# hherlyng/knp-emi-cgx

Measured on AMD Instinct MI355X. Metric: MDoF/s per implicit timestep (assembly+GMRES), higher is better.
Workload: dtype f64

## Files before the change

include/knpemi_hip.h:

```cpp
#ifndef KNPEMI_HIP_H
#define KNPEMI_HIP_H

#include <stdint.h>

#ifdef __cplusplus
extern "C" {
#endif

#define KNP_MAX_IONS 3
#define KNP_MAX_AUX 8
#define KNP_DIAG_MAX_CONSTS 64
#define KNP_MAX_PROG_REGS 48
#define KNP_STATE_MAX_INSTR 768
#define KNP_STATE_MAX_CONSTS 128
#define KNP_MAX_AMG_LEVELS 16
#define KNP_FUNCTIONAL_MAX_Q 125

#define KNP_OK 0
#define KNP_E_ARG (-1)
#define KNP_E_HIP (-2)
#define KNP_E_STATE (-3)
#define KNP_E_ALLOC (-4)
#define KNP_E_MESH (-5)

// ... 241 lines not shown
int knp_timer_read(knp_ctx* ctx, int32_t capacity, double* seconds , int32_t* n_intervals);
int knp_timer_pending(const knp_ctx* ctx);
int knp_profile_enable(knp_ctx* ctx, int32_t class_mask);
int knp_profile_get(knp_ctx* ctx, int32_t cls, double* ms, int64_t* launches);
int knp_profile_reset(knp_ctx* ctx);
enum { KNP_ST_BNORM = 0 , KNP_ST_ALLREDUCE = 1 ,
       KNP_ST_HALO = 2 , KNP_ST_READBACK = 3 ,
       KNP_ST_FUSED = 4 ,
       KNP_ST_NORM_FALLBACK = 5 ,
       KNP_ST_BLOCKED = 6 ,
       KNP_ST_FUSED_LEVELS = 7 ,
       KNP_ST_FUSED_DOTS = 8 ,
       KNP_ST_SPMV_DOTS = 9 ,
       KNP_ST_FUSED_TAILS = 10 ,
       KNP_ST_KNOD_SKIPS = 11 ,
       KNP_ST_COUNT = 12 };
int knp_get_stats(const knp_ctx* ctx, double* out );
int knp_get_traffic_model(const knp_ctx* ctx, double* out );
enum { KNP_LI_ASM_VARIANT = 0 ,
       KNP_LI_ASM_STAGE = 1 ,
       KNP_LI_ASM_DMAX = 2 ,
       KNP_LI_ASM_GROUP = 3, KNP_LI_SPMV_GROUP = 4, KNP_LI_PC_GROUP = 5 ,
       KNP_LI_MAX_NODE_CELLS = 6 ,
       KNP_LI_MAX_NODE_PAIRS = 7 ,
       KNP_LI_SPMV_UNROLL = 8 ,
       KNP_LI_SPMV_MK = 9 ,
       KNP_LI_COUNT = 10 };
int knp_get_launch_info(const knp_ctx* ctx, int32_t* out , int n);
enum { KNP_AI_A_LANES = 0, KNP_AI_P_LANES = 1, KNP_AI_R_LANES = 2, KNP_AI_S_LANES = 3, KNP_AI_RT_LANES = 4, KNP_AI_U_LANES = 5,
       KNP_AI_BA_LANES = 6, KNP_AI_BR_LANES = 7, KNP_AI_BS_LANES = 8, KNP_AI_BRT_LANES = 9, KNP_AI_BU_LANES = 10,
       KNP_AI_P_N_ACT = 11, KNP_AI_S_N_ACT = 12 ,
// ... 13 lines not shown
```

knp-emi-cgx_amd/cgx_hip/backend.py:

```python
from __future__ import annotations

import ctypes as C
import os

import numpy as np
import torch

from . import _lib
from ._lib import Fields, FieldsOut, KnpError, MeshDesc
from .parallel import HaloPlan, all_reduce_sum_, guarded


class _CAI:

    def __init__(self, ptr, n):
        self.__cuda_array_interface__ = {"shape": (int(n),), "typestr": "<f8", "data": (int(ptr), False),
                                         "version": 2, "strides": None}


def _f64(a):
    return a.ctypes.data_as(_lib.f64p)


def _i32(a):
# ... 673 lines not shown
                k = C.c_int32()
                self.check(self.lib.knp_timer_read(self.ctx, 1, out, C.byref(k)))
            return np.zeros(0)
        out = (C.c_double * n)()
        k = C.c_int32()
        self.check(self.lib.knp_timer_read(self.ctx, n, out, C.byref(k)))
        return np.array(out[:k.value], dtype=np.float64)

    def profile_enable(self, mask=0x1f):
        self.check(self.lib.knp_profile_enable(self.ctx, int(mask)))

    def profile_reset(self):
        self.check(self.lib.knp_profile_reset(self.ctx))

    def stats(self):
        out = (C.c_double * 12)()
        self.check(self.lib.knp_get_stats(self.ctx, out))
        return {"bnorm": out[0], "allreduces": int(out[1]), "halos": int(out[2]), "readbacks": int(out[3]), "fused": int(out[4]),
                "norm_fallbacks": int(out[5]), "blocked": int(out[6]), "fused_levels": int(out[7]),
                "fused_dots": int(out[8]), "spmv_dots": int(out[9]), "fused_tails": int(out[10]), "knod_skips": int(out[11])}

    def nodal_conc(self):
        out = np.empty((self.n_nodes, 4), dtype=np.float64)
        self.check(self.lib.knp_get_nodal_conc(self.ctx, _f64(out)))
        return out

    def traffic_model(self):
        out = (C.c_double * 5)()
        self.check(self.lib.knp_get_traffic_model(self.ctx, out))
        return {"spmv": out[0], "pc": out[1], "assembly_matrix": out[2], "assembly_rhs": out[3], "vector": out[4]}

    def launch_info(self):
        names = ["asm_variant", "asm_stage", "asm_dmax", "asm_group", "spmv_group", "pc_group", "max_node_cells", "max_node_pairs",
                 "spmv_unroll", "spmv_mk"]
        out = (C.c_int32 * len(names))()
# ... 21 lines not shown
```

knp-emi-cgx_amd/csrc/knp_internal.hpp:

```cpp
#pragma once
#include <hip/hip_runtime.h>

#include <cstdint>
#include <string>
#include <vector>

#include "knpemi_hip.h"

#define KNP_NPROF 5

struct KnpHostGraph {
    int dim = 0, nv1 = 0;
    int n_v = 0, n_v_owned = 0, n_c = 0, n_c_owned = 0, n_g = 0, n_q = 0;
    int n_nodes = 0, n_nodes_owned = 0;
    std::vector<int32_t> node_i, node_e;
    std::vector<int32_t> node_vertex;
    std::vector<uint8_t> node_side;
    std::vector<int32_t> pair_ptr;
    std::vector<int32_t> pair_col;
    std::vector<int32_t> pair_row;
    std::vector<double> pair_M, pair_K;
    std::vector<int32_t> contrib_ptr;
    std::vector<int32_t> contrib_cell;
    std::vector<double> contrib_k;
// ... 363 lines not shown
    bool asm_pending = false;
    double last_bnorm = 0.0;
    int64_t n_allreduce = 0, n_halo = 0, n_readback = 0;
    int64_t n_fused_dots = 0;
    int64_t n_spmv_dots = 0;
    int fused_tail = 1;
    int update_early = 1;
    bool tail_ok = false;
    bool have_tail_target = false;
    knp_fields_out tail_target = {};
    const double* tail_x = nullptr;
    bool fields_current = false, knod_current = false, fields_promise = false;
    bool knod_skipped = false;
    int64_t n_fused_tail = 0;
    int64_t n_knod_skip = 0;
    std::vector<hipEvent_t> tm_events;
    size_t tm_used = 0;
    KnpDiagMap diag_cells, diag_facets;
    KnpDiagMap diag_flux;
    double2* d_flux_rec = nullptr;
    KnpDiagMap diag_phim;
    int32_t* diag_code = nullptr;
    int diag_n_instr = 0, diag_n_regs = 0, diag_n_consts = 0;
    double diag_consts[KNP_DIAG_MAX_CONSTS] = {};
    bool diag_prog = false;
    KnpEmi emi;
    KnpStates states;
    std::vector<KnpSamplePlan> sample_plans;
    std::vector<KnpFunctional> functionals;
    std::vector<KnpFunctional> membrane_functionals;
// ... 11 lines not shown
```

knp-emi-cgx_amd/csrc/knp_kernels.hip:

```cpp
#include <hip/hip_runtime.h>
#include <hip/hip_ext.h>

#include <algorithm>
#include <cmath>
#include <cstdio>
#include <cstdlib>
#include <cstring>
#include <new>

#include "knp_dispatch.hpp"
#include "knp_internal.hpp"

#define HIPCHK(call)                                                                       \
    do {                                                                                   \
        hipError_t e_ = (call);                                                            \
        if (e_ != hipSuccess) {                                                            \
            ctx->err = std::string(#call) + ": " + hipGetErrorString(e_);                  \
            return KNP_E_HIP;                                                              \
        }                                                                                  \
    } while (0)
#define KCHK(expr)                         \
    do {                                   \
        int rc_ = (expr);                  \
        if (rc_ != KNP_OK) return rc_;     \
// ... 14 lines not shown
    double dz2i[3], dz2e[3];
    double rFz[3], cmFz[3];
    double rF;
};
struct FieldPtrs {
    const double* ki[3];
    const double* ke[3];
    const double* phim;
    const double* aux[KNP_MAX_AUX];
};

static void side_discard(knp_ctx* ctx);
static DevParams make_params(const knp_ctx* ctx);
static int64_t phi_block_nnz(const knp_ctx* ctx);
static int join_asm(knp_ctx* ctx);
static bool fin_ok(const knp_ctx* ctx);
static hipEvent_t prof_event(knp_ctx* ctx);
static void free_hier(KnpAmgHier& H);
static inline int nblocks(int64_t n, int per = NT) { return (int)std::max<int64_t>(1, (n + per - 1) / per); }

__device__ __forceinline__ double wave_sum(double v) {
#pragma unroll
    for (int o = 32; o > 0; o >>= 1) v += __shfl_xor(v, o, 64);
    return v;
}
__device__ __forceinline__ double block_sum(double v, double* sm) {
    v = wave_sum(v);
    const int w = threadIdx.x >> 6, l = threadIdx.x & 63;
    __syncthreads();
    if (l == 0) sm[w] = v;
// ... 316 lines not shown
    for (int o = G >> 1; o > 0; o >>= 1) {
        T0 += __shfl_xor(T0, o, G);
        T1 += __shfl_xor(T1, o, G);
        T2 += __shfl_xor(T2, o, G);
    }
    if (live && selfq < 255 && (selfq & (G - 1)) == lane) emit(p0 + selfq, -T0, -T1, -T2);
}

static void launch_cell_means(knp_ctx* ctx, const FieldPtrs& f, bool matrix = false) {
    const KnpHostGraph& g = ctx->g;
    bool skip = matrix && ctx->asm_dmax > 0 && ctx->fields_promise && ctx->knod_current && ctx->have_tail_target && (ctx->prof_on & ~1) == 0;
    for (int j = 0; j < 3 && skip; ++j) skip = f.ki[j] == ctx->tail_target.k_i[j] && f.ke[j] == ctx->tail_target.k_e[j];
    ctx->fields_promise = false;
    ctx->knod_current = false;
    if (matrix) ctx->knod_skipped = skip;
    if (skip) { ++ctx->n_knod_skip; return; }
    if (ctx->asm_dmax > 0)
        hipLaunchKernelGGL(k_nodal_conc, dim3(nblocks(g.n_nodes)), dim3(NT), 0, ctx->stream, g.n_nodes, ctx->d_node_vertex, ctx->d_node_side, f, ctx->d_knod);
    else
        hipLaunchKernelGGL(k_cell_means, dim3(nblocks(g.n_c)), dim3(NT), 0, ctx->stream, g.n_c, g.nv1, ctx->d_cells, ctx->d_cell_side, f, ctx->d_cbar);
}
template <bool PRECOND, bool TD_ONLY>
static void launch_assemble_nodes(knp_ctx* ctx, const DevParams& P, double* at, double* ac) {
    const KnpHostGraph& g = ctx->g;
    const int n = g.n_nodes_owned;
    if (n <= 0) return;
    if (ctx->asm_stage > 0 && ctx->d_tc_meta) {
        const int cmax = ctx->asm_stage;
        const int dmax = ctx->asm_dmax, nv1 = g.nv1;
        with_lanes<4, 32>(ctx->asm_group, [&](auto G) { with_flag(dmax > 0, [&](auto F) {
            hipLaunchKernelGGL((k_assemble_nodes_tr<PRECOND, TD_ONLY, G(), F()>), dim3(nblocks((int64_t)n * G())), dim3(NT),
// ... 2345 lines not shown
                if (nd >= g.n_nodes || g.node_vertex[nd] != v || g.node_side[nd] != s) { ok = false; break; }
                ++hits;
            }
        ctx->tail_ok = ok && hits == g.n_nodes;
    }
    std::vector<int32_t>().swap(g.contrib_cell);
    std::vector<double>().swap(g.contrib_k);
    std::vector<int32_t>().swap(g.node_cell);
    std::vector<uint8_t>().swap(g.contrib_slot);
    return KNP_OK;
}

int knp_destroy(knp_ctx* ctx) {
    if (!ctx) return KNP_OK;
    (void)hipDeviceSynchronize();
    if (ctx->stream2) { (void)hipEventDestroy(ctx->ev_fork); (void)hipEventDestroy(ctx->ev_join); (void)hipStreamDestroy(ctx->stream2); }
    if (ctx->stream3) { (void)hipEventDestroy(ctx->ev_x); (void)hipEventDestroy(ctx->ev_halo); (void)hipStreamDestroy(ctx->stream3); }
    if (ctx->stream_asm) { (void)hipEventDestroy(ctx->ev_fork_asm); (void)hipEventDestroy(ctx->ev_asm); (void)hipStreamDestroy(ctx->stream_asm); }
    dev_free(ctx->d_t2_s); dev_free(ctx->d_w2_s); dev_free(ctx->d_wb); dev_free(ctx->d_partial_s);
    dev_free(ctx->d_nodes_int); dev_free(ctx->d_nodes_bnd);
    knp_p2p_free(ctx);
    knp_jit_release(ctx);
    for (auto& r : ctx->prof_recs) { (void)hipEventDestroy(r.a); (void)hipEventDestroy(r.b); }
    for (auto& e : ctx->prof_pool) (void)hipEventDestroy(e);
    for (auto& e : ctx->tm_events) (void)hipEventDestroy(e);
    dev_free(ctx->d_cells); dev_free(ctx->d_cell_side); dev_free(ctx->d_coords);
    dev_free(ctx->d_node_vertex); dev_free(ctx->d_node_side); dev_free(ctx->d_node_i); dev_free(ctx->d_node_e);
    dev_free(ctx->d_pair_ptr); dev_free(ctx->d_pair_col); dev_free(ctx->d_pair_row);
    dev_free(ctx->d_pair_M); dev_free(ctx->d_pair_K); dev_free(ctx->d_pair_MK);
    dev_free(ctx->d_contrib_ptr); dev_free(ctx->d_contrib_cell); dev_free(ctx->d_contrib_k);
    dev_free(ctx->d_node_cell_ptr); dev_free(ctx->d_node_cell); dev_free(ctx->d_contrib_slot); dev_free(ctx->d_ncv); dev_free(ctx->d_knod);
    dev_free(ctx->d_tc_meta); dev_free(ctx->d_tc_k); dev_free(ctx->d_tc_slot);
    dev_free(ctx->d_fv); dev_free(ctx->d_fmeas); dev_free(ctx->d_gamma_prog); dev_free(ctx->d_qp); dev_free(ctx->d_qw);
    dev_free(ctx->d_gv_vertex); dev_free(ctx->d_gv_node_i); dev_free(ctx->d_gv_node_e); dev_free(ctx->d_node_gv);
    dev_free(ctx->d_gptr); dev_free(ctx->d_gcol); dev_free(ctx->d_grow); dev_free(ctx->d_gq_i); dev_free(ctx->d_gq_e);
    dev_free(ctx->d_gdiag); dev_free(ctx->d_gcptr); dev_free(ctx->d_gc_facet); dev_free(ctx->d_gc_lab);
    dev_free(ctx->d_at); dev_free(ctx->d_ac); dev_free(ctx->d_ax); dev_free(ctx->d_gx_i); dev_free(ctx->d_gx_e);
    dev_free(ctx->d_p_vals); dev_free(ctx->d_px);
    dev_free(ctx->d_cbar); dev_free(ctx->d_fmat); dev_free(ctx->d_fvec);
    dev_free(ctx->d_partial); dev_free(ctx->d_red); dev_free(ctx->d_y); dev_free(ctx->d_vbj); dev_free(ctx->d_gm);
    if (ctx->h_red) (void)hipHostFree(ctx->h_red);
    if (ctx->h_seq) (void)hipHostFree((void*)ctx->h_seq);
    dev_free(ctx->d_V); dev_free(ctx->d_Z); dev_free(ctx->d_w); dev_free(ctx->d_t);
    for (auto& p : ctx->progs) { dev_free(p.d_code); dev_free(p.d_consts); if (p.h_consts) (void)hipHostFree(p.h_consts); }
    dev_free(ctx->d_prog_code); dev_free(ctx->d_prog_consts); dev_free(ctx->d_prog_len); dev_free(ctx->d_prog_nconsts);
    for (int h = 0; h < KNP_MAX_HIER; ++h) free_hier(ctx->hier[h]);
    dev_free(ctx->d_p_vals_f);
    dev_free(ctx->d_ML); dev_free(ctx->d_cc); dev_free(ctx->d_t2); dev_free(ctx->d_w2);
    dev_free(ctx->d_defl_mode); dev_free(ctx->d_defl_einv); dev_free(ctx->d_bc_dofs);
    knp_diag_free(ctx);
    knp_emi_free(ctx);
    knp_state_free(ctx);
// ... 114 lines not shown
    HIPCHK(hipStreamSynchronize(ctx->stream));
    HIPCHK(hipMemcpy(h.data(), ctx->d_partial, h.size() * sizeof(double), hipMemcpyDeviceToHost));
    double m = 0.0;
    for (int k = 0; k < 3; ++k)
        if (len[k] > 0)
            for (int b = 0; b < RED_BLOCKS; ++b) m = std::max(m, h[(size_t)k * RED_BLOCKS + b]);
    *out = m;
    return KNP_OK;
}

int knp_set_params(knp_ctx* ctx, double dt, double F, double C_M, double psi, int32_t n_ions, const double* z,
                   const double* Di, const double* De) {
    CHECK_CTX(ctx);
    if (n_ions != 3 || !z || !Di || !De) { ctx->err = "n_ions must be 3 (Na, K, Cl; KNPEMIx_problem.py:980-981)"; return KNP_E_ARG; }
    if (!(dt > 0) || !(psi > 0) || F == 0.0) { ctx->err = "dt, psi must be positive and F non-zero"; return KNP_E_ARG; }
    ctx->dt = dt; ctx->F = F; ctx->C_M = C_M; ctx->psi = psi; ctx->n_ions = 3;
    ctx->asm_dt = -1.0;
    for (int j = 0; j < 3; ++j) {
        if (z[j] == 0.0 || !(Di[j] > 0) || !(De[j] > 0)) { ctx->err = "valence must be non-zero and diffusivities positive"; return KNP_E_ARG; }
        ctx->z[j] = z[j]; ctx->Di[j] = Di[j]; ctx->De[j] = De[j];
    }
    return KNP_OK;
}

static int validate_program(knp_ctx* ctx, int n_instr, const int32_t* code, int n_consts, int* n_regs_out) {
    int max_reg = -1;
    for (int i = 0; i < n_instr; ++i) {
        const int op = code[4 * i], d = code[4 * i + 1], a = code[4 * i + 2], b = code[4 * i + 3];
        auto regok = [&](int r) { if (r > max_reg) max_reg = r; return r >= 0 && r < KNP_MAX_PROG_REGS; };
        bool ok = true;
// ... 77 lines not shown
int knp_set_dirichlet(knp_ctx* ctx, int32_t n, const int32_t* dofs) {
    CHECK_CTX(ctx);
    side_discard(ctx);
    if (n < 0 || (n > 0 && !dofs)) { ctx->err = "bad Dirichlet arguments"; return KNP_E_ARG; }
    for (int i = 0; i < n; ++i)
        if (dofs[i] < 0 || dofs[i] >= ctx->n_dof_owned) { ctx->err = "Dirichlet dof out of range (owned dofs only)"; return KNP_E_ARG; }
    HIPCHK(hipStreamSynchronize(ctx->stream));
    dev_free(ctx->d_bc_dofs);
    ctx->n_bc = 0;
    if (n > 0) {
        KCHK(dev_upload_raw(ctx, &ctx->d_bc_dofs, dofs, (size_t)n));
        ctx->n_bc = n;
    }
    ctx->asm_dt = -1.0;
    ctx->fields_current = ctx->knod_current = false;
    return KNP_OK;
}

int knp_set_sources(knp_ctx* ctx, const double* const* fi, const double* const* fe) {
    CHECK_CTX(ctx);
    ctx->have_sources = false;
    for (int j = 0; j < 3; ++j) {
        ctx->src_i[j] = fi ? fi[j] : nullptr;
        ctx->src_e[j] = fe ? fe[j] : nullptr;
        if (ctx->src_i[j] || ctx->src_e[j]) ctx->have_sources = true;
    }
    return KNP_OK;
}

static int check_fields(knp_ctx* ctx, const knp_fields* f, bool need_phim) {
// ... 9 lines not shown
    if (ctx->pc_kind == KNP_PC_AMG || ctx->pc_kind == KNP_PC_VBJACOBI) { ctx->have_cc = false; return; }
    const KnpHostGraph& g = ctx->g;
    hipLaunchKernelGGL(k_schur_diag, dim3(nblocks(g.n_nodes_owned)), dim3(NT), 0, ctx->stream, g.n_nodes_owned, ctx->psi, ctx->z[0], ctx->z[1],
                       ctx->z[2], ctx->d_node_vertex, ctx->d_node_side, f, ctx->d_ML, ctx->d_cc);
    ctx->have_cc = true;
}

static int join_asm(knp_ctx* ctx) {
    if (ctx->asm_pending) {
        HIPCHK(hipStreamWaitEvent(ctx->stream, ctx->ev_asm, 0));
        ctx->asm_pending = false;
    }
    return KNP_OK;
}

static int assemble_matrix_on_stream(knp_ctx* ctx, const knp_fields* fields, bool with_schur_diag) {
    const KnpHostGraph& g = ctx->g;
    const DevParams P = make_params(ctx);
    FieldPtrs f = make_fields(fields);
    ProfScope ps(ctx, 3);
    launch_cell_means(ctx, f, true);
    const bool td_only = ctx->have_A && !ctx->asm_full && ctx->asm_dt == ctx->dt;
    if (td_only) launch_assemble_nodes<false, true>(ctx, P, ctx->d_at, ctx->d_ac);
    else launch_assemble_nodes<false, false>(ctx, P, ctx->d_at, ctx->d_ac);
    ctx->asm_dt = ctx->dt;
    if (g.n_g > 0) {
        if (g.dim == 2)
            hipLaunchKernelGGL((k_gamma_facets<2, true, false, 8, 1, NT, 1>), dim3(nblocks((int64_t)g.n_g * 8)), dim3(NT), 0, ctx->stream, g.n_g, g.n_q, P,
                               ctx->d_fv, ctx->d_fmeas, ctx->d_qp, ctx->d_qw, f, 0, ctx->d_coords, ctx->d_gamma_prog,
                               (const int32_t* const*)nullptr, (const int32_t*)nullptr, (const double* const*)nullptr,
                               (const int32_t*)nullptr, 0, 0, ctx->d_fmat, ctx->d_fvec);
        else if (gamma_many(g)) {
            hipLaunchKernelGGL((k_gamma_facets<3, true, false, 4, 9, 64, 1>), dim3((unsigned)(((int64_t)g.n_g * 4 + 63) / 64)), dim3(64), 0, ctx->stream, g.n_g, g.n_q, P,
                               ctx->d_fv, ctx->d_fmeas, ctx->d_qp, ctx->d_qw, f, 0, ctx->d_coords, ctx->d_gamma_prog,
                               (const int32_t* const*)nullptr, (const int32_t*)nullptr, (const double* const*)nullptr,
                               (const int32_t*)nullptr, 0, 0, ctx->d_fmat, ctx->d_fvec);
        }
        else
            hipLaunchKernelGGL((k_gamma_facets<3, true, false, 16, 3, 64, 2>), dim3((unsigned)(((int64_t)g.n_g * 16 + 63) / 64)), dim3(64), 0, ctx->stream, g.n_g, g.n_q, P,
                               ctx->d_fv, ctx->d_fmeas, ctx->d_qp, ctx->d_qw, f, 0, ctx->d_coords, ctx->d_gamma_prog,
                               (const int32_t* const*)nullptr, (const int32_t*)nullptr, (const double* const*)nullptr,
                               (const int32_t*)nullptr, 0, 0, ctx->d_fmat, ctx->d_fvec);
        if (ctx->n_gp)
            hipLaunchKernelGGL((k_gamma_pairs<false>), dim3(nblocks(ctx->n_gp)), dim3(NT), 0, ctx->stream, ctx->n_gp, g.n_g, g.dim, P,
                               ctx->d_grow, ctx->d_gptr, ctx->d_gv_node_i, ctx->d_gv_node_e, ctx->d_gq_i, ctx->d_gq_e,
                               ctx->d_gcptr, ctx->d_gc_facet, ctx->d_gc_lab, ctx->d_fmeas, ctx->d_fmat, ctx->d_pair_ptr,
                               ctx->d_at, ctx->d_ax);
    }
    if (ctx->n_bc > 0)
        hipLaunchKernelGGL(k_dirichlet_rows_A, dim3(nblocks(ctx->n_bc)), dim3(NT), 0, ctx->stream, ctx->n_bc, ctx->d_bc_dofs, ctx->d_pair_ptr,
                           ctx->d_pair_col, ctx->d_node_gv, ctx->d_node_side, ctx->d_gptr, ctx->d_ac, ctx->d_at, ctx->d_ax);
    if (with_schur_diag && !ctx->prep.left()) launch_schur_diag(ctx, f);
    HIPCHK(hipGetLastError());
    ctx->have_A = true;
    if (ctx->pc_kind == KNP_PC_VBJACOBI) {
        hipLaunchKernelGGL(k_vbj_extract, dim3(nblocks(g.n_nodes_owned)), dim3(NT), 0, ctx->stream, g.n_nodes_owned,
                           ctx->d_pair_ptr, ctx->d_pair_col, ctx->d_ac, ctx->d_at, ctx->d_ax, ctx->d_node_gv, ctx->d_node_side,
                           ctx->d_gdiag, ctx->d_vbj);
        HIPCHK(hipGetLastError());
    }
    return KNP_OK;
}

int knp_assemble_matrix(knp_ctx* ctx, const knp_fields* fields) {
    CHECK_CTX(ctx);
    KCHK(check_fields(ctx, fields, false));
    KCHK(join_asm(ctx));
    return assemble_matrix_on_stream(ctx, fields, true);
}

int knp_assemble_matrix_async(knp_ctx* ctx, const knp_fields* fields) {
    CHECK_CTX(ctx);
    KCHK(check_fields(ctx, fields, false));
    KCHK(join_asm(ctx));
    static const bool off = getenv("KNP_ASM_ASYNC") && atoi(getenv("KNP_ASM_ASYNC")) == 0;
    if (off || ctx->pc_kind == KNP_PC_VBJACOBI || (ctx->prof_on & ~1) || !ctx->have_A || ctx->prep.left())
        return assemble_matrix_on_stream(ctx, fields, true);
    if (!ctx->stream_asm) {
        HIPCHK(hipStreamCreateWithFlags(&ctx->stream_asm, hipStreamNonBlocking));
        HIPCHK(hipEventCreateWithFlags(&ctx->ev_fork_asm, hipEventDisableTiming));
        HIPCHK(hipEventCreateWithFlags(&ctx->ev_asm, hipEventDisableTiming));
    }
    HIPCHK(hipEventRecord(ctx->ev_fork_asm, ctx->stream));
    HIPCHK(hipStreamWaitEvent(ctx->stream_asm, ctx->ev_fork_asm, 0));
    hipStream_t main_stream = ctx->stream;
    ctx->stream = ctx->stream_asm;
    const int rc = assemble_matrix_on_stream(ctx, fields, false);
    ctx->stream = main_stream;
    KCHK(rc);
    HIPCHK(hipEventRecord(ctx->ev_asm, ctx->stream_asm));
    ctx->asm_pending = true;
    return KNP_OK;
}

int knp_pc_set_coupled_potential(knp_ctx* ctx, int32_t on) {
    CHECK_CTX(ctx);
    side_discard(ctx);
    ctx->pc_coupled_phi = on ? 1 : 0;
    if (on && !ctx->d_px) {
        HIPCHK(hipMalloc((void**)&ctx->d_px, (size_t)std::max<int64_t>(ctx->n_gp, 1) * sizeof(double)));
        HIPCHK(hipMemset(ctx->d_px, 0, (size_t)std::max<int64_t>(ctx->n_gp, 1) * sizeof(double)));
    }
// ... 27 lines not shown
        rp[n] = (int32_t)k;
        for (int p = g.pair_ptr[n]; p < g.pair_ptr[n + 1]; ++p) { ci[k] = g.pair_col[p]; vals[k++] = pm[(size_t)4 * p + 3]; }
        const int A = g.node_gv[n];
        if (ctx->pc_coupled_phi && A >= 0) {
            const std::vector<int32_t>& gx = g.node_side[n] ? g.gx_e : g.gx_i;
            for (int s = g.gptr[A]; s < g.gptr[A + 1]; ++s) { ci[k] = gx[s]; vals[k++] = px[s]; }
        }
    }
    rp[g.n_nodes_owned] = (int32_t)k;
    return KNP_OK;
}

int knp_assemble_precond(knp_ctx* ctx, const knp_fields* fields) {
    CHECK_CTX(ctx);
    side_discard(ctx);
    KCHK(join_asm(ctx));
    KCHK(check_fields(ctx, fields, false));
    const KnpHostGraph& g = ctx->g;
    const DevParams P = make_params(ctx);
    FieldPtrs f = make_fields(fields);
    ProfScope ps(ctx, 3);
    launch_cell_means(ctx, f);
    launch_assemble_nodes<true, false>(ctx, P, ctx->d_p_vals, nullptr);
    if (g.n_g > 0 && ctx->n_gp)
        hipLaunchKernelGGL((k_gamma_pairs<true>), dim3(nblocks(ctx->n_gp)), dim3(NT), 0, ctx->stream, ctx->n_gp, g.n_g, g.dim, P,
                           ctx->d_grow, ctx->d_gptr, ctx->d_gv_node_i, ctx->d_gv_node_e, ctx->d_gq_i, ctx->d_gq_e,
                           ctx->d_gcptr, ctx->d_gc_facet, ctx->d_gc_lab, ctx->d_fmeas, ctx->d_fmat, ctx->d_pair_ptr,
                           ctx->d_p_vals, nullptr, ctx->pc_coupled_phi ? ctx->d_px : nullptr);
    if (ctx->n_bc > 0)
        hipLaunchKernelGGL(k_dirichlet_rows_P, dim3(nblocks(ctx->n_bc)), dim3(NT), 0, ctx->stream, ctx->n_bc, ctx->d_bc_dofs, ctx->d_pair_ptr,
// ... 161 lines not shown
    if (cnt <= 0) return KNP_OK;
    const int no = ctx->g.n_nodes_owned;
    const int nb = std::min(RED_BLOCKS, nblocks(no));
    hipLaunchKernelGGL(k_phi_sum, dim3(nb), dim3(NT), 0, ctx->stream, no, v, ctx->d_partial);
    hipLaunchKernelGGL(k_reduce_partials, dim3(1), dim3(NT), 0, ctx->stream, nb, ctx->d_partial, ctx->d_red, 62, (double*)nullptr);
    KCHK(allreduce_slots(ctx, 62, 1));
    hipLaunchKernelGGL(k_phi_sub, dim3(nblocks(no)), dim3(NT), 0, ctx->stream, no, ctx->d_red + 62, 1.0 / (double)cnt, v);
    HIPCHK(hipGetLastError());
    return KNP_OK;
}
int knp_project_nullspace(knp_ctx* ctx, double* v) {
    CHECK_CTX(ctx);
    side_discard(ctx);
    if (!v) return KNP_E_ARG;
    ctx->fields_current = ctx->knod_current = false;
    return project_ns(ctx, v);
}

static int ensure_work(knp_ctx* ctx, int restart) {
    if (!ctx->d_w) {
        HIPCHK(hipMalloc((void**)&ctx->d_w, std::max(ctx->n_dof_local, 1) * sizeof(double)));
        HIPCHK(hipMalloc((void**)&ctx->d_t, std::max(ctx->n_dof_local, 1) * sizeof(double)));
        HIPCHK(hipMemset(ctx->d_w, 0, std::max(ctx->n_dof_local, 1) * sizeof(double)));
        HIPCHK(hipMemset(ctx->d_t, 0, std::max(ctx->n_dof_local, 1) * sizeof(double)));
    }
    if (restart > 0 && (ctx->gm_restart < restart || !ctx->d_V)) {
        HIPCHK(hipStreamSynchronize(ctx->stream));
        dev_free(ctx->d_V);
        size_t bytes = (size_t)(restart + 1) * std::max(ctx->n_dof_local, 1) * sizeof(double);
        HIPCHK(hipMalloc((void**)&ctx->d_V, bytes));
// ... 817 lines not shown
        KCHK(check_hier(ctx, 0));
        KCHK(check_hier(ctx, 1));
        if (!ctx->d_t2) {
            HIPCHK(hipMalloc((void**)&ctx->d_t2, std::max(ctx->n_dof_local, 1) * sizeof(double)));
            HIPCHK(hipMalloc((void**)&ctx->d_w2, std::max(ctx->n_dof_local, 1) * sizeof(double)));
            HIPCHK(hipMemset(ctx->d_t2, 0, std::max(ctx->n_dof_local, 1) * sizeof(double)));
            HIPCHK(hipMemset(ctx->d_w2, 0, std::max(ctx->n_dof_local, 1) * sizeof(double)));
        }
    }
    ctx->pc_kind = kind;
    ctx->fused_dots = !(getenv("KNP_FUSED_DOTS") && atoi(getenv("KNP_FUSED_DOTS")) == 0);
    ctx->spmv_dots = !(getenv("KNP_SPMV_DOTS") && atoi(getenv("KNP_SPMV_DOTS")) == 0);
    ctx->gmres_ahead = !(getenv("KNP_GMRES_AHEAD") && atoi(getenv("KNP_GMRES_AHEAD")) == 0);
    ctx->fused_tail = !(getenv("KNP_FUSED_TAIL") && atoi(getenv("KNP_FUSED_TAIL")) == 0);
    ctx->update_early = !(getenv("KNP_UPDATE_EARLY") && atoi(getenv("KNP_UPDATE_EARLY")) == 0);
    ctx->fields_current = ctx->knod_current = false;
    for (int h = 0; h < KNP_MAX_HIER; ++h) ctx->hier[h].fused = 0;
    if (kind == KNP_PC_AMG) ctx->hier[0].fused = fused_eligible(ctx, ctx->hier[0]) ? 1 : 0;
    if (kind == KNP_PC_AMG_BT || kind == KNP_PC_AMG_LT) {
        const bool ok = fused_eligible(ctx, ctx->hier[0]) && fused_eligible(ctx, ctx->hier[1]) && ctx->hier[1].native0 == 3 && ctx->hier[0].native0 == 2 &&
                        ctx->hier[1].lv[0].S_n_act > 0 && ctx->hier[1].lv[0].S_act_rows_c && ctx->hier[1].lv[0].R_ci_c;
        ctx->hier[0].fused = ctx->hier[1].fused = ok ? 1 : 0;
        if (!ok && ctx->hier[1].l0_upload) ctx->hier[1].native0 = 0;
    }
    for (int h = 0; h < KNP_MAX_HIER; ++h) {
        KnpAmgHier& H = ctx->hier[h];
        const bool off = getenv("KNP_BLOCKED") && atoi(getenv("KNP_BLOCKED")) == 0;
        bool ok = !off && H.fused && H.node_nf > 0 && (H.native0 == 1 || H.native0 == 2) && (H.native0 == 1) == (H.node_nf == 4);
        for (int l = 0; ok && l < H.levels - 1; ++l) {
            const KnpAmgLevel& L = H.lv[l];
            ok = L.bR.rp && L.bS.rp && (l == 0 || L.bA.rp) && L.bR.n_rows * H.node_nf == L.n_coarse &&
// ... 182 lines not shown
    }
    if (!f->phi_i || !f->phi_e || (need_phim && !f->phi_m)) { ctx->err = "null potential field"; return KNP_E_ARG; }
    o.phi_i = f->phi_i; o.phi_e = f->phi_e; o.phi_m = f->phi_m;
    return KNP_OK;
}
static bool same_target(const knp_ctx* ctx, const knp_fields_out* f) {
    if (!ctx->have_tail_target) return false;
    const knp_fields_out& t = ctx->tail_target;
    for (int j = 0; j < 3; ++j)
        if (f->k_i[j] != t.k_i[j] || f->k_e[j] != t.k_e[j]) return false;
    return f->phi_i == t.phi_i && f->phi_e == t.phi_e && f->phi_m == t.phi_m;
}
int knp_set_unpack_target(knp_ctx* ctx, const knp_fields_out* f) {
    CHECK_CTX(ctx);
    ctx->fields_current = ctx->knod_current = ctx->fields_promise = false;
    ctx->have_tail_target = false;
    if (!f) return KNP_OK;
    OutPtrs o;
    KCHK(out_ptrs(ctx, f, o, true));
    ctx->tail_target = *f;
    ctx->have_tail_target = true;
    return KNP_OK;
}
int knp_fields_unchanged(knp_ctx* ctx) {
    CHECK_CTX(ctx);
    ctx->fields_promise = true;
    return KNP_OK;
}
int knp_get_nodal_conc(knp_ctx* ctx, double* out) {
    CHECK_CTX(ctx);
    if (!out) return KNP_E_ARG;
    if (ctx->asm_dmax <= 0 || !ctx->d_knod) { ctx->err = "this context's assembly keeps no node-indexed concentration copy"; return KNP_E_STATE; }
    KCHK(join_asm(ctx));
    HIPCHK(hipStreamSynchronize(ctx->stream));
    HIPCHK(hipMemcpy(out, ctx->d_knod, (size_t)4 * ctx->g.n_nodes * sizeof(double), hipMemcpyDeviceToHost));
    return KNP_OK;
}
int knp_pack(knp_ctx* ctx, const knp_fields_out* f, double* x) {
    CHECK_CTX(ctx);
    if (!x) return KNP_E_ARG;
    OutPtrs o;
    KCHK(out_ptrs(ctx, f, o, false));
    ctx->fields_current = ctx->knod_current = false;
    hipLaunchKernelGGL(k_pack, dim3(nblocks(ctx->g.n_nodes)), dim3(NT), 0, ctx->stream, ctx->g.n_nodes, ctx->d_node_vertex,
                       ctx->d_node_side, o, x);
    HIPCHK(hipGetLastError());
    return KNP_OK;
}
int knp_unpack(knp_ctx* ctx, const double* x, const knp_fields_out* f) {
    CHECK_CTX(ctx);
    if (!x) return KNP_E_ARG;
    OutPtrs o;
    KCHK(out_ptrs(ctx, f, o, true));
    if (ctx->fields_current && x == ctx->tail_x && same_target(ctx, f)) return KNP_OK;
    ctx->fields_current = ctx->knod_current = false;
    KCHK(join_asm(ctx));
    KCHK(halo_update(ctx, const_cast<double*>(x)));
    hipLaunchKernelGGL(k_unpack, dim3(nblocks(ctx->g.n_v)), dim3(NT), 0, ctx->stream, ctx->g.n_v, ctx->d_node_i, ctx->d_node_e, x, o);
    HIPCHK(hipGetLastError());
    return KNP_OK;
}
int knp_hh_update(knp_ctx* ctx, const double* phi_m, double* n, double* m, double* h, int32_t count, double dt, double phi_rest,
                  int32_t rush_larsen, int32_t substeps) {
    CHECK_CTX(ctx);
    if (!phi_m || !n || !m || !h || count < 0 || substeps < 1 || !(dt > 0)) { ctx->err = "bad hh_update arguments"; return KNP_E_ARG; }
    if (count == 0) return KNP_OK;
    ProfScope ps(ctx, 4);
    hipLaunchKernelGGL(k_hh_update, dim3(nblocks(count)), dim3(NT), 0, ctx->stream, count, phi_m, n, m, h, dt, phi_rest,
                       rush_larsen, substeps);
    HIPCHK(hipGetLastError());
// ... 57 lines not shown
    CHECK_CTX(ctx);
    if (cls < 0 || cls >= KNP_NPROF || !ms || !launches) return KNP_E_ARG;
    KCHK(prof_collect(ctx));
    *ms = ctx->prof_ms[cls];
    *launches = ctx->prof_n[cls];
    return KNP_OK;
}
int knp_profile_reset(knp_ctx* ctx) {
    CHECK_CTX(ctx);
    KCHK(prof_collect(ctx));
    for (int i = 0; i < KNP_NPROF; ++i) { ctx->prof_ms[i] = 0; ctx->prof_n[i] = 0; }
    ctx->n_allreduce = ctx->n_halo = ctx->n_readback = ctx->n_norm_fallback = 0;
    ctx->n_fused_dots = 0;
    ctx->n_spmv_dots = 0;
    ctx->n_fused_tail = ctx->n_knod_skip = 0;
    return KNP_OK;
}
static double cycle_bytes(const knp_ctx* ctx, const KnpAmgHier& H) {
    if (H.levels < 1) return 0.0;
    const double vs = H.cinv_f || ctx->amg_fp32 ? 4.0 : 8.0;
    double b = 0.0;
    const int nl = H.levels;
    const int nf0 = H.native0 == 1 ? 4 : H.native0 == 2 ? 3 : 1;
    const double n0 = (double)ctx->g.n_nodes_owned;
    auto blocked = [&](const KnpBlockedCsr& M, int nf) { return (double)M.nnz * (nf == 4 ? 20.0 : 16.0) + 4.0 * (M.n_rows + 1); };
    auto scalar = [&](int64_t nnz, int rows) { return (double)nnz * (vs + 4.0) + 4.0 * (rows + 1); };
    if (H.at0_rp) b += scalar(H.lv[0].A_nnz, ctx->g.n_nodes_owned);
    else if (H.native0) b += (double)ctx->n_pairs * (vs * nf0 + 4.0) + 4.0 * (n0 + 1);
    else b += scalar(H.lv[0].A_nnz, H.lv[0].n);
    b += 8.0 * n0 * nf0 * 3.0;
// ... 39 lines not shown
    out[KNP_ST_BNORM] = ctx->last_bnorm;
    out[KNP_ST_ALLREDUCE] = (double)ctx->n_allreduce;
    out[KNP_ST_HALO] = (double)ctx->n_halo;
    out[KNP_ST_READBACK] = (double)ctx->n_readback;
    out[KNP_ST_FUSED] = (double)(ctx->hier[0].fused + 2 * ctx->hier[1].fused + 4 * ctx->hier[0].l0_fused + 8 * ctx->hier[1].l0_fused);
    out[KNP_ST_NORM_FALLBACK] = (double)ctx->n_norm_fallback;
    out[KNP_ST_BLOCKED] = (double)(ctx->hier[0].blocked + 2 * ctx->hier[1].blocked);
    int nlf = 0;
    for (int h = 0; h < KNP_MAX_HIER; ++h)
        for (int l = 1; l < ctx->hier[h].levels; ++l) nlf += ctx->hier[h].lv[l].lfused;
    out[KNP_ST_FUSED_LEVELS] = (double)nlf;
    out[KNP_ST_FUSED_DOTS] = (double)ctx->n_fused_dots;
    out[KNP_ST_SPMV_DOTS] = (double)ctx->n_spmv_dots;
    out[KNP_ST_FUSED_TAILS] = (double)ctx->n_fused_tail;
    out[KNP_ST_KNOD_SKIPS] = (double)ctx->n_knod_skip;
    return KNP_OK;
}
int knp_get_launch_info(const knp_ctx* ctx, int32_t* out, int n) {
    if (!ctx || !out || n <= 0) return KNP_E_ARG;
    const KnpHostGraph& g = ctx->g;
    int32_t v[KNP_LI_COUNT];
    v[KNP_LI_ASM_VARIANT] = ctx->asm_stage > 0 ? (ctx->d_tc_meta ? 2 : 1) : 0;
    v[KNP_LI_ASM_STAGE] = ctx->asm_stage;
    v[KNP_LI_ASM_DMAX] = ctx->asm_dmax;
    v[KNP_LI_ASM_GROUP] = ctx->asm_group;
    v[KNP_LI_SPMV_GROUP] = ctx->spmv_group;
    v[KNP_LI_PC_GROUP] = ctx->pc_group;
    v[KNP_LI_MAX_NODE_CELLS] = g.max_node_cells;
    int dmax = 0;
    if ((int)g.pair_ptr.size() > g.n_nodes_owned)
// ... 57 lines not shown
```

knp-emi-cgx_amd/csrc/knp_krylov.inc:

```

static constexpr int GM_RES = 100, GM_EXPL = 57, GM_MAX_RESTART = GM_EXPL - 2;
static constexpr int FB_SLOT = 124;
static_assert(GM_RES + 2 <= RED_SLOTS && DEFL_SLOT0 + DEFL_MAX <= GM_RES, "reduction slot layout");
static constexpr double GM_DTOL = 1e5;

static void side_discard(knp_ctx* ctx) {
    switch (ctx->prep.kind) {
        case KnpSidePrep::NONE:
        case KnpSidePrep::LEFT_DEFERRED: break;
        default: (void)hipEventSynchronize(ctx->ev_join);
    }
    ctx->prep.kind = KnpSidePrep::NONE;
}
static int ensure_side_stream(knp_ctx* ctx) {
    if (ctx->stream2) return KNP_OK;
    HIPCHK(hipStreamCreateWithFlags(&ctx->stream2, hipStreamNonBlocking));
    HIPCHK(hipEventCreateWithFlags(&ctx->ev_fork, hipEventDisableTiming));
    HIPCHK(hipEventCreateWithFlags(&ctx->ev_join, hipEventDisableTiming));
    return KNP_OK;
}

static bool exchanges_all_native(const knp_ctx* ctx) {
    if (!ctx->p2p || ctx->p2p_fine < 0 || ctx->p2p_red < 0 || ctx->defl_m > 0) return false;
    const int nh = ctx->pc_kind == KNP_PC_AMG ? 1 : (ctx->pc_kind == KNP_PC_AMG_BT || ctx->pc_kind == KNP_PC_AMG_LT) ? 2 : 0;
// ... 187 lines not shown
    int nb, vec_blocks;
    bool ns;
    double inv_cnt;
    double ttol, atol, dref;
};

static int krylov_begin(knp_ctx* ctx, const double* b, double* x, int32_t max_it, int32_t restart, int32_t* its, double* rnorm, int32_t* reason,
                        bool flexible, KrylovSolve* K, int64_t* cnt) {
    if (!b || !x || !its || !rnorm || !reason) return KNP_E_ARG;
    if (!ctx->have_A) { ctx->err = "matrix not assembled"; return KNP_E_STATE; }
    if (restart < 1 || restart > GM_MAX_RESTART || max_it < 0) {
        ctx->err = "restart must be in [1," + std::to_string(GM_MAX_RESTART) + "] and max_it >= 0";
        return KNP_E_ARG;
    }
    ctx->fields_current = ctx->knod_current = false;
    KCHK(ensure_work(ctx, restart));
    if (flexible && ctx->pc_kind != KNP_PC_NONE) KCHK(ensure_z(ctx, restart));
    prof_collect_ready(ctx);
    int rc;
    *cnt = ctx->ns_on ? global_phi_count(ctx, &rc) : 0;
    if (ctx->ns_on) KCHK(rc);
    const GmLayout GL{restart};
    if (ctx->gm_cap < GL.size()) {
        HIPCHK(hipStreamSynchronize(ctx->stream));
        dev_free(ctx->d_gm);
        HIPCHK(hipMalloc((void**)&ctx->d_gm, (size_t)GL.size() * sizeof(double)));
        HIPCHK(hipMemset(ctx->d_gm, 0, (size_t)GL.size() * sizeof(double)));
        ctx->gm_cap = GL.size();
    }
    const int n = ctx->n_dof_owned;
// ... 247 lines not shown
            else KCHK(enqueue_iteration(j, ctx->update_early ? K.ttol : 0.0));
            KCHK(arnoldi_step_read(K, j, ctx->d_V + (size_t)(j + 1) * ldv, &res, &flag, have));
            if (krylov_stop_test(K, j, flag, res, max_it, &it, &jd, reason)) { stop = true; break; }
        }
        if (jd > 0) {
            ProfScope ps(ctx, 1);
            if (stop && tail_ok && jd <= 8) {
                OutPtrs o;
                KCHK(out_ptrs(ctx, &ctx->tail_target, o, true));
                hipLaunchKernelGGL(k_lincomb_unpack, dim3(nblocks(ctx->g.n_v)), dim3(NT), 0, st, GL, jd, gm, ctx->g.n_v, ldv, ctx->d_V, x, ctx->d_node_i,
                                   ctx->d_node_e, o, ctx->asm_dmax > 0 ? ctx->d_knod : nullptr);
                ctx->tail_x = x;
                ctx->fields_current = true;
                ctx->knod_current = ctx->asm_dmax > 0;
                ++ctx->n_fused_tail;
            } else {
                krylov_update_plain(K, jd, ctx->d_V, x);
            }
        }
        if (stop) break;
    }
    return krylov_end(K, x, it, res, its, rnorm);
}

int knp_fgmres_solve(knp_ctx* ctx, const double* b, double* x, double rtol, double atol, int32_t max_it, int32_t restart,
                     int32_t* its, double* rnorm, int32_t* reason) {
    CHECK_CTX(ctx);
    KrylovSolve K;
    int64_t cnt;
    KCHK(krylov_begin(ctx, b, x, max_it, restart, its, rnorm, reason, true, &K, &cnt));
// ... 83 lines not shown
```

Before: 2245.

## Speculatively assemble next-step matrix on side stream after GMRES fused tail

When the GMRES solve ends through the fused unpack tail, the next timestep's matrix is launched early on the assembly stream into alternate buffers, using the freshly unpacked fields. The next assemble call adopts it by swapping buffers if the field pointers and dt match, and otherwise discards it. This overlaps matrix assembly with host-side work between timesteps and skips recomputing cell means. In exchange it costs extra device memory for the double buffers, and the speculation is wasted whenever the eligibility conditions are not met.

```diff
diff --git a/include/knpemi_hip.h b/include/knpemi_hip.h
--- a/include/knpemi_hip.h
+++ b/include/knpemi_hip.h
@@ -279,7 +279,9 @@
        KNP_ST_SPMV_DOTS = 9 ,
        KNP_ST_FUSED_TAILS = 10 ,
        KNP_ST_KNOD_SKIPS = 11 ,
-       KNP_ST_COUNT = 12 };
+       KNP_ST_AHEAD_ADOPTED = 12 ,
+       KNP_ST_AHEAD_DISCARDED = 13 ,
+       KNP_ST_COUNT = 14 };
 int knp_get_stats(const knp_ctx* ctx, double* out );
 int knp_get_traffic_model(const knp_ctx* ctx, double* out );
 enum { KNP_LI_ASM_VARIANT = 0 ,
diff --git a/knp-emi-cgx_amd/cgx_hip/backend.py b/knp-emi-cgx_amd/cgx_hip/backend.py
--- a/knp-emi-cgx_amd/cgx_hip/backend.py
+++ b/knp-emi-cgx_amd/cgx_hip/backend.py
@@ -711,11 +711,12 @@
         self.check(self.lib.knp_profile_reset(self.ctx))
 
     def stats(self):
-        out = (C.c_double * 12)()
+        out = (C.c_double * 14)()
         self.check(self.lib.knp_get_stats(self.ctx, out))
         return {"bnorm": out[0], "allreduces": int(out[1]), "halos": int(out[2]), "readbacks": int(out[3]), "fused": int(out[4]),
                 "norm_fallbacks": int(out[5]), "blocked": int(out[6]), "fused_levels": int(out[7]),
-                "fused_dots": int(out[8]), "spmv_dots": int(out[9]), "fused_tails": int(out[10]), "knod_skips": int(out[11])}
+                "fused_dots": int(out[8]), "spmv_dots": int(out[9]), "fused_tails": int(out[10]), "knod_skips": int(out[11]),
+                "asm_ahead": int(out[12]), "asm_ahead_discarded": int(out[13])}
 
     def nodal_conc(self):
         out = np.empty((self.n_nodes, 4), dtype=np.float64)
diff --git a/knp-emi-cgx_amd/csrc/knp_internal.hpp b/knp-emi-cgx_amd/csrc/knp_internal.hpp
--- a/knp-emi-cgx_amd/csrc/knp_internal.hpp
+++ b/knp-emi-cgx_amd/csrc/knp_internal.hpp
@@ -401,6 +401,18 @@
     bool knod_skipped = false;
     int64_t n_fused_tail = 0;
     int64_t n_knod_skip = 0;
+    int asm_ahead = 1;
+    bool asm_armed = false;
+    bool asm_alt_failed = false;
+    double *d_at_alt = nullptr, *d_ax_alt = nullptr;
+    struct AsmAhead {
+        bool pending = false;
+        const double* k_i[3] = {nullptr, nullptr, nullptr};
+        const double* k_e[3] = {nullptr, nullptr, nullptr};
+        const double* phi_m = nullptr;
+        double dt = 0.0;
+    } ahead;
+    int64_t n_ahead_adopted = 0, n_ahead_discarded = 0;
     std::vector<hipEvent_t> tm_events;
     size_t tm_used = 0;
     KnpDiagMap diag_cells, diag_facets;
diff --git a/knp-emi-cgx_amd/csrc/knp_kernels.hip b/knp-emi-cgx_amd/csrc/knp_kernels.hip
--- a/knp-emi-cgx_amd/csrc/knp_kernels.hip
+++ b/knp-emi-cgx_amd/csrc/knp_kernels.hip
@@ -52,6 +52,8 @@
 static DevParams make_params(const knp_ctx* ctx);
 static int64_t phi_block_nnz(const knp_ctx* ctx);
 static int join_asm(knp_ctx* ctx);
+static int drop_ahead(knp_ctx* ctx);
+static int speculate_asm(knp_ctx* ctx);
 static bool fin_ok(const knp_ctx* ctx);
 static hipEvent_t prof_event(knp_ctx* ctx);
 static void free_hier(KnpAmgHier& H);
@@ -398,7 +400,7 @@
     ctx->fields_promise = false;
     ctx->knod_current = false;
     if (matrix) ctx->knod_skipped = skip;
-    if (skip) { ++ctx->n_knod_skip; return; }
+    if (skip) { ++ctx->n_knod_skip; ctx->asm_armed = true; return; }
     if (ctx->asm_dmax > 0)
         hipLaunchKernelGGL(k_nodal_conc, dim3(nblocks(g.n_nodes)), dim3(NT), 0, ctx->stream, g.n_nodes, ctx->d_node_vertex, ctx->d_node_side, f, ctx->d_knod);
     else
@@ -2774,6 +2776,7 @@
 int knp_destroy(knp_ctx* ctx) {
     if (!ctx) return KNP_OK;
     (void)hipDeviceSynchronize();
+    if (ctx->stream_asm) (void)hipStreamSynchronize(ctx->stream_asm);
     if (ctx->stream2) { (void)hipEventDestroy(ctx->ev_fork); (void)hipEventDestroy(ctx->ev_join); (void)hipStreamDestroy(ctx->stream2); }
     if (ctx->stream3) { (void)hipEventDestroy(ctx->ev_x); (void)hipEventDestroy(ctx->ev_halo); (void)hipStreamDestroy(ctx->stream3); }
     if (ctx->stream_asm) { (void)hipEventDestroy(ctx->ev_fork_asm); (void)hipEventDestroy(ctx->ev_asm); (void)hipStreamDestroy(ctx->stream_asm); }
@@ -2795,7 +2798,7 @@
     dev_free(ctx->d_gv_vertex); dev_free(ctx->d_gv_node_i); dev_free(ctx->d_gv_node_e); dev_free(ctx->d_node_gv);
     dev_free(ctx->d_gptr); dev_free(ctx->d_gcol); dev_free(ctx->d_grow); dev_free(ctx->d_gq_i); dev_free(ctx->d_gq_e);
     dev_free(ctx->d_gdiag); dev_free(ctx->d_gcptr); dev_free(ctx->d_gc_facet); dev_free(ctx->d_gc_lab);
-    dev_free(ctx->d_at); dev_free(ctx->d_ac); dev_free(ctx->d_ax); dev_free(ctx->d_gx_i); dev_free(ctx->d_gx_e);
+    dev_free(ctx->d_at); dev_free(ctx->d_ac); dev_free(ctx->d_ax); dev_free(ctx->d_at_alt); dev_free(ctx->d_ax_alt); dev_free(ctx->d_gx_i); dev_free(ctx->d_gx_e);
     dev_free(ctx->d_p_vals); dev_free(ctx->d_px);
     dev_free(ctx->d_cbar); dev_free(ctx->d_fmat); dev_free(ctx->d_fvec);
     dev_free(ctx->d_partial); dev_free(ctx->d_red); dev_free(ctx->d_y); dev_free(ctx->d_vbj); dev_free(ctx->d_gm);
@@ -2940,6 +2943,7 @@
     CHECK_CTX(ctx);
     if (n_ions != 3 || !z || !Di || !De) { ctx->err = "n_ions must be 3 (Na, K, Cl; KNPEMIx_problem.py:980-981)"; return KNP_E_ARG; }
     if (!(dt > 0) || !(psi > 0) || F == 0.0) { ctx->err = "dt, psi must be positive and F non-zero"; return KNP_E_ARG; }
+    KCHK(drop_ahead(ctx));
     ctx->dt = dt; ctx->F = F; ctx->C_M = C_M; ctx->psi = psi; ctx->n_ions = 3;
     ctx->asm_dt = -1.0;
     for (int j = 0; j < 3; ++j) {
@@ -3047,6 +3051,7 @@
     }
     ctx->asm_dt = -1.0;
     ctx->fields_current = ctx->knod_current = false;
+    KCHK(drop_ahead(ctx));
     return KNP_OK;
 }
 
@@ -3086,15 +3091,15 @@
     return KNP_OK;
 }
 
-static int assemble_matrix_on_stream(knp_ctx* ctx, const knp_fields* fields, bool with_schur_diag) {
+static int assemble_matrix_on_stream(knp_ctx* ctx, const knp_fields* fields, bool with_schur_diag, double* at, double* ax, bool knod_ready = false) {
     const KnpHostGraph& g = ctx->g;
     const DevParams P = make_params(ctx);
     FieldPtrs f = make_fields(fields);
     ProfScope ps(ctx, 3);
-    launch_cell_means(ctx, f, true);
+    if (!knod_ready) launch_cell_means(ctx, f, true);
     const bool td_only = ctx->have_A && !ctx->asm_full && ctx->asm_dt == ctx->dt;
-    if (td_only) launch_assemble_nodes<false, true>(ctx, P, ctx->d_at, ctx->d_ac);
-    else launch_assemble_nodes<false, false>(ctx, P, ctx->d_at, ctx->d_ac);
+    if (td_only) launch_assemble_nodes<false, true>(ctx, P, at, ctx->d_ac);
+    else launch_assemble_nodes<false, false>(ctx, P, at, ctx->d_ac);
     ctx->asm_dt = ctx->dt;
     if (g.n_g > 0) {
         if (g.dim == 2)
@@ -3117,47 +3122,129 @@
             hipLaunchKernelGGL((k_gamma_pairs<false>), dim3(nblocks(ctx->n_gp)), dim3(NT), 0, ctx->stream, ctx->n_gp, g.n_g, g.dim, P,
                                ctx->d_grow, ctx->d_gptr, ctx->d_gv_node_i, ctx->d_gv_node_e, ctx->d_gq_i, ctx->d_gq_e,
                                ctx->d_gcptr, ctx->d_gc_facet, ctx->d_gc_lab, ctx->d_fmeas, ctx->d_fmat, ctx->d_pair_ptr,
-                               ctx->d_at, ctx->d_ax);
+                               at, ax);
     }
     if (ctx->n_bc > 0)
         hipLaunchKernelGGL(k_dirichlet_rows_A, dim3(nblocks(ctx->n_bc)), dim3(NT), 0, ctx->stream, ctx->n_bc, ctx->d_bc_dofs, ctx->d_pair_ptr,
-                           ctx->d_pair_col, ctx->d_node_gv, ctx->d_node_side, ctx->d_gptr, ctx->d_ac, ctx->d_at, ctx->d_ax);
+                           ctx->d_pair_col, ctx->d_node_gv, ctx->d_node_side, ctx->d_gptr, ctx->d_ac, at, ax);
     if (with_schur_diag && !ctx->prep.left()) launch_schur_diag(ctx, f);
     HIPCHK(hipGetLastError());
     ctx->have_A = true;
     if (ctx->pc_kind == KNP_PC_VBJACOBI) {
         hipLaunchKernelGGL(k_vbj_extract, dim3(nblocks(g.n_nodes_owned)), dim3(NT), 0, ctx->stream, g.n_nodes_owned,
-                           ctx->d_pair_ptr, ctx->d_pair_col, ctx->d_ac, ctx->d_at, ctx->d_ax, ctx->d_node_gv, ctx->d_node_side,
+                           ctx->d_pair_ptr, ctx->d_pair_col, ctx->d_ac, at, ax, ctx->d_node_gv, ctx->d_node_side,
                            ctx->d_gdiag, ctx->d_vbj);
         HIPCHK(hipGetLastError());
     }
     return KNP_OK;
 }
 
-int knp_assemble_matrix(knp_ctx* ctx, const knp_fields* fields) {
-    CHECK_CTX(ctx);
-    KCHK(check_fields(ctx, fields, false));
-    KCHK(join_asm(ctx));
-    return assemble_matrix_on_stream(ctx, fields, true);
-}
-
-int knp_assemble_matrix_async(knp_ctx* ctx, const knp_fields* fields) {
-    CHECK_CTX(ctx);
-    KCHK(check_fields(ctx, fields, false));
-    KCHK(join_asm(ctx));
+static bool ahead_form_ok(const knp_ctx* ctx) {
+    return ctx->asm_ahead && ctx->have_A && !ctx->asm_full && ctx->asm_dt == ctx->dt && ctx->n_bc == 0 && !ctx->halo && !ctx->allreduce &&
+           !ctx->level_comm && !ctx->p2p && (ctx->pc_kind == KNP_PC_AMG || ctx->pc_kind == KNP_PC_AMG_BT || ctx->pc_kind == KNP_PC_AMG_LT) &&
+           (ctx->prof_on & ~1) == 0;
+}
+static bool asm_async_off() {
     static const bool off = getenv("KNP_ASM_ASYNC") && atoi(getenv("KNP_ASM_ASYNC")) == 0;
-    if (off || ctx->pc_kind == KNP_PC_VBJACOBI || (ctx->prof_on & ~1) || !ctx->have_A || ctx->prep.left())
-        return assemble_matrix_on_stream(ctx, fields, true);
+    return off;
+}
+static int ensure_asm_stream(knp_ctx* ctx) {
     if (!ctx->stream_asm) {
         HIPCHK(hipStreamCreateWithFlags(&ctx->stream_asm, hipStreamNonBlocking));
         HIPCHK(hipEventCreateWithFlags(&ctx->ev_fork_asm, hipEventDisableTiming));
         HIPCHK(hipEventCreateWithFlags(&ctx->ev_asm, hipEventDisableTiming));
     }
+    return KNP_OK;
+}
+static int drop_ahead(knp_ctx* ctx) {
+    if (!ctx->ahead.pending) return KNP_OK;
+    ctx->ahead.pending = false;
+    ctx->asm_armed = false;
+    ++ctx->n_ahead_discarded;
+    return join_asm(ctx);
+}
+static int speculate_asm(knp_ctx* ctx) {
+    if (!ctx->asm_armed || !ahead_form_ok(ctx) || !ctx->knod_current || !ctx->have_tail_target || ctx->asm_pending || ctx->ahead.pending ||
+        ctx->prep.left() || ctx->asm_alt_failed || asm_async_off())
+        return KNP_OK;
+    if (ctx->asm_ahead < 2 && 84.0 * (double)ctx->n_pairs + 128.0 * (double)ctx->n_gp > 256.0 * 1048576.0) return KNP_OK;
+    KCHK(ensure_asm_stream(ctx));
+    if (!ctx->d_at_alt) {
+        const size_t nat = (size_t)std::max<int64_t>(4 * ctx->n_pairs, 2) * sizeof(double), nax = (size_t)std::max<int64_t>(8 * ctx->n_gp, 2) * sizeof(double);
+        if (hipMalloc((void**)&ctx->d_at_alt, nat) != hipSuccess || hipMalloc((void**)&ctx->d_ax_alt, nax) != hipSuccess) {
+            (void)hipGetLastError();
+            dev_free(ctx->d_at_alt); dev_free(ctx->d_ax_alt);
+            ctx->asm_alt_failed = true;
+            return KNP_OK;
+        }
+        HIPCHK(hipMemsetAsync(ctx->d_at_alt, 0xff, nat, ctx->stream_asm));
+        HIPCHK(hipMemsetAsync(ctx->d_ax_alt, 0xff, nax, ctx->stream_asm));
+    }
+    knp_fields f = {};
+    for (int j = 0; j < 3; ++j) { f.k_i[j] = ctx->tail_target.k_i[j]; f.k_e[j] = ctx->tail_target.k_e[j]; }
+    f.phi_m = ctx->tail_target.phi_m;
     HIPCHK(hipEventRecord(ctx->ev_fork_asm, ctx->stream));
     HIPCHK(hipStreamWaitEvent(ctx->stream_asm, ctx->ev_fork_asm, 0));
     hipStream_t main_stream = ctx->stream;
     ctx->stream = ctx->stream_asm;
-    const int rc = assemble_matrix_on_stream(ctx, fields, false);
+    const int rc = assemble_matrix_on_stream(ctx, &f, false, ctx->d_at_alt, ctx->d_ax_alt, true);
+    ctx->stream = main_stream;
+    KCHK(rc);
+    HIPCHK(hipEventRecord(ctx->ev_asm, ctx->stream_asm));
+    ctx->asm_pending = true;
+    ctx->ahead.pending = true;
+    for (int j = 0; j < 3; ++j) { ctx->ahead.k_i[j] = f.k_i[j]; ctx->ahead.k_e[j] = f.k_e[j]; }
+    ctx->ahead.phi_m = f.phi_m;
+    ctx->ahead.dt = ctx->dt;
+    return KNP_OK;
+}
+static int adopt_ahead(knp_ctx* ctx, const knp_fields* fields, bool* adopted) {
+    *adopted = false;
+    if (!ctx->ahead.pending) return KNP_OK;
+    bool ok = ctx->fields_promise && ctx->knod_current && ahead_form_ok(ctx) && ctx->ahead.dt == ctx->dt && fields->phi_m == ctx->ahead.phi_m;
+    for (int j = 0; j < 3 && ok; ++j) ok = fields->k_i[j] == ctx->ahead.k_i[j] && fields->k_e[j] == ctx->ahead.k_e[j];
+    if (!ok) return drop_ahead(ctx);
+    std::swap(ctx->d_at, ctx->d_at_alt);
+    std::swap(ctx->d_ax, ctx->d_ax_alt);
+    ctx->ahead.pending = false;
+    ctx->fields_promise = false;
+    ctx->knod_current = false;
+    ctx->knod_skipped = true;
+    ++ctx->n_knod_skip;
+    ++ctx->n_ahead_adopted;
+    *adopted = true;
+    return KNP_OK;
+}
+
+int knp_assemble_matrix(knp_ctx* ctx, const knp_fields* fields) {
+    CHECK_CTX(ctx);
+    KCHK(check_fields(ctx, fields, false));
+    bool adopted = false;
+    KCHK(adopt_ahead(ctx, fields, &adopted));
+    KCHK(join_asm(ctx));
+    if (adopted) {
+        if (!ctx->prep.left()) launch_schur_diag(ctx, make_fields(fields));
+        HIPCHK(hipGetLastError());
+        return KNP_OK;
+    }
+    return assemble_matrix_on_stream(ctx, fields, true, ctx->d_at, ctx->d_ax);
+}
+
+int knp_assemble_matrix_async(knp_ctx* ctx, const knp_fields* fields) {
+    CHECK_CTX(ctx);
+    KCHK(check_fields(ctx, fields, false));
+    bool adopted = false;
+    KCHK(adopt_ahead(ctx, fields, &adopted));
+    if (adopted) return KNP_OK;
+    KCHK(join_asm(ctx));
+    if (asm_async_off() || ctx->pc_kind == KNP_PC_VBJACOBI || (ctx->prof_on & ~1) || !ctx->have_A || ctx->prep.left())
+        return assemble_matrix_on_stream(ctx, fields, true, ctx->d_at, ctx->d_ax);
+    KCHK(ensure_asm_stream(ctx));
+    HIPCHK(hipEventRecord(ctx->ev_fork_asm, ctx->stream));
+    HIPCHK(hipStreamWaitEvent(ctx->stream_asm, ctx->ev_fork_asm, 0));
+    hipStream_t main_stream = ctx->stream;
+    ctx->stream = ctx->stream_asm;
+    const int rc = assemble_matrix_on_stream(ctx, fields, false, ctx->d_at, ctx->d_ax);
     ctx->stream = main_stream;
     KCHK(rc);
     HIPCHK(hipEventRecord(ctx->ev_asm, ctx->stream_asm));
@@ -3215,6 +3302,7 @@
 int knp_assemble_precond(knp_ctx* ctx, const knp_fields* fields) {
     CHECK_CTX(ctx);
     side_discard(ctx);
+    KCHK(drop_ahead(ctx));
     KCHK(join_asm(ctx));
     KCHK(check_fields(ctx, fields, false));
     const KnpHostGraph& g = ctx->g;
@@ -3406,6 +3494,7 @@
     side_discard(ctx);
     if (!v) return KNP_E_ARG;
     ctx->fields_current = ctx->knod_current = false;
+    KCHK(drop_ahead(ctx));
     return project_ns(ctx, v);
 }
 
@@ -4253,7 +4342,9 @@
     ctx->gmres_ahead = !(getenv("KNP_GMRES_AHEAD") && atoi(getenv("KNP_GMRES_AHEAD")) == 0);
     ctx->fused_tail = !(getenv("KNP_FUSED_TAIL") && atoi(getenv("KNP_FUSED_TAIL")) == 0);
     ctx->update_early = !(getenv("KNP_UPDATE_EARLY") && atoi(getenv("KNP_UPDATE_EARLY")) == 0);
+    ctx->asm_ahead = getenv("KNP_ASM_AHEAD") ? std::max(atoi(getenv("KNP_ASM_AHEAD")), 0) : 1;
     ctx->fields_current = ctx->knod_current = false;
+    KCHK(drop_ahead(ctx));
     for (int h = 0; h < KNP_MAX_HIER; ++h) ctx->hier[h].fused = 0;
     if (kind == KNP_PC_AMG) ctx->hier[0].fused = fused_eligible(ctx, ctx->hier[0]) ? 1 : 0;
     if (kind == KNP_PC_AMG_BT || kind == KNP_PC_AMG_LT) {
@@ -4466,6 +4557,7 @@
 int knp_set_unpack_target(knp_ctx* ctx, const knp_fields_out* f) {
     CHECK_CTX(ctx);
     ctx->fields_current = ctx->knod_current = ctx->fields_promise = false;
+    KCHK(drop_ahead(ctx));
     ctx->have_tail_target = false;
     if (!f) return KNP_OK;
     OutPtrs o;
@@ -4494,6 +4586,7 @@
     OutPtrs o;
     KCHK(out_ptrs(ctx, f, o, false));
     ctx->fields_current = ctx->knod_current = false;
+    KCHK(drop_ahead(ctx));
     hipLaunchKernelGGL(k_pack, dim3(nblocks(ctx->g.n_nodes)), dim3(NT), 0, ctx->stream, ctx->g.n_nodes, ctx->d_node_vertex,
                        ctx->d_node_side, o, x);
     HIPCHK(hipGetLastError());
@@ -4506,6 +4599,7 @@
     KCHK(out_ptrs(ctx, f, o, true));
     if (ctx->fields_current && x == ctx->tail_x && same_target(ctx, f)) return KNP_OK;
     ctx->fields_current = ctx->knod_current = false;
+    KCHK(drop_ahead(ctx));
     KCHK(join_asm(ctx));
     KCHK(halo_update(ctx, const_cast<double*>(x)));
     hipLaunchKernelGGL(k_unpack, dim3(nblocks(ctx->g.n_v)), dim3(NT), 0, ctx->stream, ctx->g.n_v, ctx->d_node_i, ctx->d_node_e, x, o);
@@ -4593,6 +4687,7 @@
     ctx->n_fused_dots = 0;
     ctx->n_spmv_dots = 0;
     ctx->n_fused_tail = ctx->n_knod_skip = 0;
+    ctx->n_ahead_adopted = ctx->n_ahead_discarded = 0;
     return KNP_OK;
 }
 static double cycle_bytes(const knp_ctx* ctx, const KnpAmgHier& H) {
@@ -4662,6 +4757,8 @@
     out[KNP_ST_SPMV_DOTS] = (double)ctx->n_spmv_dots;
     out[KNP_ST_FUSED_TAILS] = (double)ctx->n_fused_tail;
     out[KNP_ST_KNOD_SKIPS] = (double)ctx->n_knod_skip;
+    out[KNP_ST_AHEAD_ADOPTED] = (double)ctx->n_ahead_adopted;
+    out[KNP_ST_AHEAD_DISCARDED] = (double)ctx->n_ahead_discarded;
     return KNP_OK;
 }
 int knp_get_launch_info(const knp_ctx* ctx, int32_t* out, int n) {
diff --git a/knp-emi-cgx_amd/csrc/knp_krylov.inc b/knp-emi-cgx_amd/csrc/knp_krylov.inc
--- a/knp-emi-cgx_amd/csrc/knp_krylov.inc
+++ b/knp-emi-cgx_amd/csrc/knp_krylov.inc
@@ -225,6 +225,7 @@
         return KNP_E_ARG;
     }
     ctx->fields_current = ctx->knod_current = false;
+    KCHK(drop_ahead(ctx));
     KCHK(ensure_work(ctx, restart));
     if (flexible && ctx->pc_kind != KNP_PC_NONE) KCHK(ensure_z(ctx, restart));
     prof_collect_ready(ctx);
@@ -502,6 +503,7 @@
                 ctx->fields_current = true;
                 ctx->knod_current = ctx->asm_dmax > 0;
                 ++ctx->n_fused_tail;
+                KCHK(speculate_asm(ctx));
             } else {
                 krylov_update_plain(K, jd, ctx->d_V, x);
             }
```

After: 2299 (median of 6 runs). +2.4%, better.
